# heiheishuang/MuDG

Hardware: AMD Instinct MI355X
Metric: DDIM denoise steps/sec, MDM1024 576x1024x16f (CFG: 2 UNet forwards + fused update per step, per clip) (higher is better)
Workload: dtype bf16; 1 GPU; MDM1024 latents (B=1,4,16,72,128) + c_concat 8ch, context (B,333,1024), 50-step uniform_trailing DDIM schedule, cfg 7.5, guidance_rescale 0.7, eta 1.0, v-prediction, dynamic rescale; clips_per_gpu=1, parallelism=clip-DP x1 (no in-step collective), launch=hipGraph replay of each UNet pass (cond+uncond batched)

## Files before the change

### include/mudg_hip.h

```cpp
#ifndef MUDG_HIP_H
#define MUDG_HIP_H

#include <stdint.h>

#ifdef __cplusplus
extern "C" {
#endif

#define MUDG_OK          0
#define MUDG_EINVAL     -1
#define MUDG_ELAUNCH    -2
#define MUDG_EUNSUPPORTED -3

int mudg_version(void);
int mudg_operand_dtype(void);
const char* mudg_last_error(void);

typedef struct MudgGemmDesc {
    const void* X;
    const void* X2;
    const void* W;
    void*       Y;
    const float* bias;
    const float* gbias;
// ... 35 lines not shown
    int Nk2, ldk2, ldvt2, kv_div2;
    int64_t svt2;
    const void* Q8; const void* K8; const void* Qs; const void* Ks;
    int ldq8, ldk8, ldqs, ldks;
    int q_prescaled;
    float* Lse;
} MudgAttnDesc;
int mudg_attention(const MudgAttnDesc* d, void* stream);
int mudg_quantize_mxfp8(const void* X, int ldx, int64_t rows, int cols, void* Y8, int ldy, void* S, int lds, void* stream);

int mudg_temporal_attention(const void* QKV, void* O, int B, int T, int HW, int heads,
                            int ldqkv, int ldo, float scale, void* stream);
int mudg_temporal_self_attention_ok(int T, int HW, int heads, int C, int64_t ldx, int64_t ldw, int64_t ldo);
int mudg_temporal_self_attention(const void* X, const void* Wh, void* O, int B, int T, int HW, int heads, int C, int64_t ldx,
                                 int64_t ldw, int64_t ldo, float scale, void* stream);

int64_t mudg_groupnorm_ws_floats(int samples, int groups, int rows);
int mudg_groupnorm(const void* X, const void* X2, int csplit, int ldx, int ldx2, int x_fp32,
                   const float* gamma, const float* beta, void* Y, int ldy,
                   int samples, int rows, int C, int groups, float eps, int silu,
                   float* ws, void* stream);
int mudg_groupnorm_fused(const void* X, const void* X2, int csplit, int ldx, int ldx2, int x_fp32,
                         const float* gamma, const float* beta, void* Y, int ldy,
                         int samples, int rows, int C, int groups, float eps, int silu,
                         const float* P1, const float* P2, float* ws, void* stream);

int mudg_groupnorm_fused_rows(const void* X, const void* X2, int csplit, int ldx, int ldx2, int x_fp32,
                              const float* gamma, const float* beta, void* Y, int ldy,
                              int samples, int rows, int C, int groups, float eps, int silu,
                              const float* P1, int p1_rows, const float* P2, int p2_rows, float* ws, void* stream);
// ... 200 lines not shown
```

### mudg_amd/csrc/attention.hip

```cpp
#include "attn_shared.h"
#include <cstdlib>

namespace {

#if MUDG_PLANES == 1
template <bool TWO>
__global__ __launch_bounds__(256, 2) void attn_kernel(const MudgAttnDesc p, const int nqt, const int total) {
    __shared__ __attribute__((aligned(16))) h16 Ks[2 * ATILE];
    __shared__ __attribute__((aligned(16))) h16 Vs[2 * ATILE];

    const int tid = threadIdx.x, lane = tid & 63, wave = tid >> 6;
    const int l31 = lane & 31, hi = lane >> 5;

    const int w = xcd_work_item(total);
    const int pair = w / nqt, qt = w - pair * nqt;
    const int f = pair / p.heads, h = pair - f * p.heads;
    const h16* Qp = reinterpret_cast<const h16*>(p.Q) + (int64_t)f * p.Nq * p.ldq + h * 64;
    h16* Op = reinterpret_cast<h16*>(p.O) + (int64_t)f * p.Nq * p.ldo + h * 64;

    const int q = qt * QB + wave * 32 + l31;
    const bool qok = q < p.Nq;

    h16x8 qf[1][4];
    load_q_frags(qf[0], Qp, q, p.ldq, 0, qok, hi);
// ... 18 lines not shown

        for (int kt = 0; kt < nkt; ++kt) {
            const int cur = kt & 1;
            const bool more = kt + 1 < nkt;
            if (more) load_kv_tile(kv, kt + 1, lrow, kc, kr, vr);
            FLASH_TILE(Ks + cur * ATILE, Vs + cur * ATILE, qf, kt, kv.Nk, c, m_run, l_run, o, l31, hi);
            if (more) stage_padded(Ks + (cur ^ 1) * ATILE, Vs + (cur ^ 1) * ATILE, lrow, kc, kr, vr);
            __syncthreads();
        }
        inv = finish_set<TWO>(p, set, f, h, q, qok, hi, c, m_run, l_run, o, res);
    }
    if (qok) store_o16(o, inv, Op + (int64_t)q * p.ldo, hi, p.accumulate);
}

constexpr int XK_TILES = 3;
template <bool TWO>
__global__ __launch_bounds__(256, 2) void xattn_kernel(const MudgAttnDesc p, const int nqt, const int xq, const int nqc, const int total) {
    extern __shared__ __attribute__((aligned(16))) h16 xlds[];
    h16* Ks = xlds;
    h16* Vs = xlds + XK_TILES * ATILE;
    const int tid = threadIdx.x, lane = tid & 63, wave = tid >> 6;
    const int l31 = lane & 31, hi = lane >> 5;
    const int w = xcd_work_item(total);
    const int pair = w / nqc, qc = w - pair * nqc;
    const int f = pair / p.heads, h = pair - f * p.heads;
    const h16* Qp = reinterpret_cast<const h16*>(p.Q) + (int64_t)f * p.Nq * p.ldq + h * 64;
    h16* Op = reinterpret_cast<h16*>(p.O) + (int64_t)f * p.Nq * p.ldo + h * 64;
    const int nt0 = (p.Nk + KB - 1) / KB;

    {
        const int lrow = tid >> 3, kc = tid & 7;
#pragma unroll
// ... 17 lines not shown
        const int q = qt * QB + wave * 32 + l31;
        const bool qok = q < p.Nq;
        h16x8 qf[1][4];
        load_q_frags(qf[0], Qp, q, p.ldq, 0, qok, hi);
        f32x16 o[2], res[TWO ? 2 : 1];
        float inv = 0.f;
#pragma unroll
        for (int set = 0; set < (TWO ? 2 : 1); ++set) {
            const int Nk = set == 0 ? p.Nk : p.Nk2;
#pragma unroll
            for (int r = 0; r < 16; ++r) { o[0][r] = 0.f; o[1][r] = 0.f; }
            float m_run = -INFINITY, l_run = 0.f;
            const int nkt = (Nk + KB - 1) / KB;
            for (int kt = 0; kt < nkt; ++kt) {
                const int ti = set == 0 ? kt : nt0 + kt;
                FLASH_TILE(Ks + ti * ATILE, Vs + ti * ATILE, qf, kt, Nk, c, m_run, l_run, o, l31, hi);
            }
            inv = finish_set<TWO>(p, set, f, h, q, qok, hi, c, m_run, l_run, o, res);
        }
        if (qok) store_o16(o, inv, Op + (int64_t)q * p.ldo, hi, p.accumulate);
    }
}

__global__ __launch_bounds__(256, 2) void attn64q_kernel(const MudgAttnDesc p, const int nqt, const int total) {
    __shared__ __attribute__((aligned(16))) h16 Ks[2 * ATILE];
    __shared__ __attribute__((aligned(16))) h16 Vs[2 * ATILE];

    const int tid = threadIdx.x, lane = tid & 63, wave = tid >> 6;
    const int l31 = lane & 31, hi = lane >> 5;
    const int w = xcd_work_item(total);
    const int pair = w / nqt, qt = w - pair * nqt;
    const int f = pair / p.heads, h = pair - f * p.heads;
    const KvSet kv = kv_set(p, f, h, 0);

    const h16* Qp = reinterpret_cast<const h16*>(p.Q) + (int64_t)f * p.Nq * p.ldq + h * 64;
    h16* Op = reinterpret_cast<h16*>(p.O) + (int64_t)f * p.Nq * p.ldo + h * 64;
// ... 374 lines not shown
        if (rok) {
            h16* dst = O + row * ldo + h * 64 + dp * DW;
#pragma unroll
            for (int i = 0; i < DW / 8; ++i) {
                h16x8 t;
#pragma unroll
                for (int e = 0; e < 8; ++e) t[e] = (h16)ov[i * 8 + e];
                st16(dst + i * 8, as_u32x4(t));
            }
        }
    }
}


#if MUDG_PLANES == 1
#ifdef MUDG_OPERAND_FP16
typedef __attribute__((ext_vector_type(4))) _Float16 mf4;
#define MFMA_16x16x32(a, b, c) __builtin_amdgcn_mfma_f32_16x16x32_f16(a, b, c, 0, 0, 0)
#define MFMA_16x16x16(a, b, c) __builtin_amdgcn_mfma_f32_16x16x16f16(a, b, c, 0, 0, 0)
#else
typedef __attribute__((ext_vector_type(4))) short mf4;
#define MFMA_16x16x32(a, b, c) __builtin_amdgcn_mfma_f32_16x16x32_bf16(a, b, c, 0, 0, 0)
#define MFMA_16x16x16(a, b, c) __builtin_amdgcn_mfma_f32_16x16x16bf16_1k(a, b, c, 0, 0, 0)
#endif

__device__ __forceinline__ int tattn_fz(int rg) { return (rg & 1) | ((rg >> 1) << 3); }
__device__ __forceinline__ void tattn_item_mfma(const char* qs, const char* ks, const char* vs, const int c, const int g, const int T,
                                                const float scale, float (&ov)[16]) {
    f32x4 st = {0.f, 0.f, 0.f, 0.f};
#pragma unroll
    for (int s = 0; s < 2; ++s) {
        const int off = c * 128 + (((g + 4 * s) ^ (c & 7)) << 4);
        st = MFMA_16x16x32(as_h16x8(ld16(ks + off)), as_h16x8(ld16(qs + off)), st);
    }

    float sc[4];
    float mx = -INFINITY;
#pragma unroll
    for (int i = 0; i < 4; ++i) { sc[i] = (4 * g + i < T) ? st[i] * scale : -INFINITY; mx = fmaxf(mx, sc[i]); }
// ... 680 lines not shown
        }
        else if (dma_ok && d.q_prescaled && lean) hipLaunchKernelGGL((attn64d_kernel<true, false>), dim3((unsigned)total2), dim3(256), 0, s, d, nqt2, (int)total2);
        else if (dma_ok) hipLaunchKernelGGL((attn64d_kernel<false, false>), dim3((unsigned)total2), dim3(256), 0, s, d, nqt2, (int)total2);
        else hipLaunchKernelGGL(attn64q_kernel, dim3((unsigned)total2), dim3(256), 0, s, d, nqt2, (int)total2);
    } else {
        static int xv = -1;
        if (xv < 0) xv = mudg_variant("ATTN_X", 1);
        int xq = (int)(total / 1024);
        xq = xq > 8 ? 8 : xq;
        if (xv && xq >= 2 && d.Nk <= 2 * KB && (!d.K2 || d.Nk2 <= KB)) {
            constexpr int smem = 2 * XK_TILES * ATILE * (int)sizeof(h16);
            if (const int rc = mudg_lds_opt_in<&xattn_kernel<false>>(smem, "mudg_attention")) return rc;
            if (const int rc = mudg_lds_opt_in<&xattn_kernel<true>>(smem, "mudg_attention")) return rc;
            const int nqc = (nqt + xq - 1) / xq;
            const int64_t totx = (int64_t)nqc * d.F * d.heads;
            if (d.K2) hipLaunchKernelGGL(xattn_kernel<true>, dim3((unsigned)totx), dim3(256), smem, s, d, nqt, xq, nqc, (int)totx);
            else hipLaunchKernelGGL(xattn_kernel<false>, dim3((unsigned)totx), dim3(256), smem, s, d, nqt, xq, nqc, (int)totx);
        }
        else if (d.K2) hipLaunchKernelGGL(attn_kernel<true>, dim3((unsigned)total), dim3(256), 0, s, d, nqt, (int)total);
        else hipLaunchKernelGGL(attn_kernel<false>, dim3((unsigned)total), dim3(256), 0, s, d, nqt, (int)total);
    }
#endif
    const int rc = mudg_check_launch("mudg_attention");
    const double bh = (double)d.F * d.heads;
    mudg_prof_end(slot, s, 4.0 * bh * d.Nq * (double)(d.Nk + (d.K2 ? d.Nk2 : 0)) * 64.0,
                  bh * (2.0 * d.Nq + 2.0 * d.Nk / d.kv_div + (d.K2 ? 2.0 * d.Nk2 / d.kv_div2 : 0.0)) * 64.0 * 2.0);
    return rc;
}

#if MUDG_PLANES == 1
namespace {
__global__ __launch_bounds__(256) void quantize_mxfp8_kernel(const h16* __restrict__ X, int ldx, int64_t rows, int nblk,
// ... 107 lines not shown
    const int rc0 = mudg_lds_opt_in<tsattn_fused_kernel>(TSA_LDS, "mudg_temporal_self_attention");
    if (rc0 != MUDG_OK) return rc0;
    hipStream_t s = reinterpret_cast<hipStream_t>(stream);
    const int slot = mudg_prof_begin(MUDG_FAM_GEMM, s);
    hipLaunchKernelGGL(tsattn_fused_kernel, dim3((unsigned)total), dim3(256), TSA_LDS, s, (const h16*)X, (const h16*)Wh, (h16*)O, HW, heads, C,
                       ldx, ldw, ldo, scale, (int)total);
    const int rc = mudg_check_launch("mudg_temporal_self_attention");
    const double M = (double)B * T * HW;
    mudg_prof_end(slot, s, 2.0 * M * 3.0 * C * C + 4.0 * (double)B * HW * heads * T * T * 64.0, (2.0 * M * C + 3.0 * C * C) * 2.0);
    return rc;
#else
    (void)X; (void)Wh; (void)O; (void)B; (void)T; (void)HW; (void)heads; (void)C; (void)ldx; (void)ldw; (void)ldo; (void)scale; (void)stream;
    MUDG_FAIL(MUDG_EUNSUPPORTED, "mudg_temporal_self_attention: the fused kernel belongs to the 16-bit operand builds");
#endif
}
```

### mudg_amd/csrc/attn_shared.h

```cpp
#pragma once
#include "common.h"
#include <type_traits>

constexpr int QB = 128;
constexpr int KB = 64;
constexpr int ALD = 72;
constexpr int ATILE = 64 * ALD;

struct KvSet {
    const h16* Kp;
    const h16* Vp;
    int Nk, ldk, ldvt;
    int psk, psv;
};
__device__ __forceinline__ KvSet kv_set(const MudgAttnDesc& p, int f, int h, int set) {
    KvSet kv;
    if (set == 0) {
        kv.Kp = reinterpret_cast<const h16*>(p.K) + (int64_t)(f / p.kv_div) * p.Nk * p.ldk + h * 64;
        kv.Vp = reinterpret_cast<const h16*>(p.Vt) + (int64_t)(f / p.kv_div) * p.svt + (int64_t)(h * 64) * p.ldvt;
        kv.Nk = p.Nk; kv.ldk = p.ldk; kv.ldvt = p.ldvt;
    } else {
        kv.Kp = reinterpret_cast<const h16*>(p.K2) + (int64_t)(f / p.kv_div2) * p.Nk2 * p.ldk2 + h * 64;
        kv.Vp = reinterpret_cast<const h16*>(p.Vt2) + (int64_t)(f / p.kv_div2) * p.svt2 + (int64_t)(h * 64) * p.ldvt2;
        kv.Nk = p.Nk2; kv.ldk = p.ldk2; kv.ldvt = p.ldvt2;
// ... 29 lines not shown
                }
            }
            vr[pl][i] = v;
        }
}
__device__ __forceinline__ void stage_padded(h16* Kt, h16* Vt, int lrow, int kc, const u32x4 (&kr)[PLANES][2], const u32x4 (&vr)[PLANES][2]) {
#pragma unroll
    for (int pl = 0; pl < PLANES; ++pl)
#pragma unroll
        for (int i = 0; i < 2; ++i) {
            st16(&Kt[pl * ATILE + (lrow + 32 * i) * ALD + kc * 8], kr[pl][i]);
            st16(&Vt[pl * ATILE + (lrow + 32 * i) * ALD + kc * 8], vr[pl][i]);
        }
}

__device__ __forceinline__ void mask_ragged(f32x16 (&s)[2], int kt, int Nk, int hi) {
    if (kt * KB + KB > Nk) {
#pragma unroll
        for (int sub = 0; sub < 2; ++sub)
#pragma unroll
            for (int r = 0; r < 16; ++r) {
                const int j = kt * KB + sub * 32 + (r & 3) + 8 * (r >> 2) + 4 * hi;
                if (j >= Nk) s[sub][r] = -INFINITY;
            }
    }
}

__device__ __forceinline__ float row_max32(const f32x16 (&s)[2]) {
    float mx = s[0][0];
#pragma unroll
    for (int r = 1; r < 16; ++r) mx = fmaxf(mx, s[0][r]);
#pragma unroll
    for (int r = 0; r < 16; ++r) mx = fmaxf(mx, s[1][r]);
    return fmaxf(mx, __shfl_xor(mx, 32, 64));
}

__device__ __forceinline__ void put_p(h16x8 (&pk)[PLANES][2][2], int sub, int r, float e) {
    h16 piece[PLANES];
    split_operand(e, piece);
#pragma unroll
    for (int pl = 0; pl < PLANES; ++pl) pk[pl][sub][r >> 3][r & 7] = piece[pl];
}

__device__ __forceinline__ void softmax_step_classic(const f32x16 (&s)[2], float c, float& m_run, float& l_run, f32x16 (&o)[2],
                                                     h16x8 (&pk)[PLANES][2][2]) {
    const float mx = row_max32(s);
    const bool grew = !__all(mx <= m_run);
    const float m_new = grew ? fmaxf(m_run, mx) : m_run;
    const float alpha = grew ? __builtin_amdgcn_exp2f((m_run - m_new) * c) : 1.0f;
    const float mc = m_new * c;
    m_run = m_new;
    float ps = 0.f;
#pragma unroll
    for (int sub = 0; sub < 2; ++sub)
#pragma unroll
        for (int r = 0; r < 16; ++r) {
            const float e = __builtin_amdgcn_exp2f(fmaf(s[sub][r], c, -mc));
            ps += e;
            put_p(pk, sub, r, e);
        }
    l_run = l_run * alpha + ps;
    if (grew) {
#pragma unroll
        for (int r = 0; r < 16; ++r) { o[0][r] *= alpha; o[1][r] *= alpha; }
    }
}

#ifdef MUDG_OPERAND_FP16
constexpr float LEAN_LIMIT = 32768.f;
// ... 11 lines not shown
            put_p(pk, sub, r, e);
        }
    l_run += ps;
    return !(ps <= LEAN_LIMIT);
}
template <bool LEAN, class KeyLoop>
__device__ __forceinline__ void lean_or_classic(const bool& overflow, KeyLoop key_loop) {
    if constexpr (LEAN) {
        key_loop(std::true_type{});
        if (__syncthreads_or(overflow ? 1 : 0)) key_loop(std::false_type{});
    } else {
        key_loop(std::false_type{});
    }
}

#define FLASH_TILE(Kt, Vt, qf, kt, Nk, c, m_run, l_run, o, l31, hi) do {                                                  \
    const h16* const ft_K = (Kt); const h16* const ft_V = (Vt); const int ft_kt = (kt), ft_Nk = (Nk);                     \
    f32x16 ft_s[2];                                                                                                       \
    _Pragma("unroll") for (int sub = 0; sub < 2; ++sub) {                                                                 \
        _Pragma("unroll") for (int r = 0; r < 16; ++r) ft_s[sub][r] = 0.f;                                                \
        _Pragma("unroll") for (int sg = 0; sg < NSEG; ++sg) {                                                             \
            const h16* kp = ft_K + seg_xp(sg) * ATILE + (sub * 32 + (l31)) * ALD + (hi) * 8;                              \
            _Pragma("unroll") for (int ks = 0; ks < 4; ++ks) {                                                            \
                const h16x8 kf = *reinterpret_cast<const h16x8*>(kp + ks * 16);                                           \
                ft_s[sub] = MFMA_32x32x16(kf, (qf)[seg_wp(sg)][ks], ft_s[sub]);                                           \
            }                                                                                                             \
        }                                                                                                                 \
    }                                                                                                                     \
    mask_ragged(ft_s, ft_kt, ft_Nk, (hi));                                                                                \
    h16x8 ft_pk[PLANES][2][2];                                                                                            \
    softmax_step_classic(ft_s, (c), (m_run), (l_run), (o), ft_pk);                                                        \
    _Pragma("unroll") for (int dt = 0; dt < 2; ++dt)                                                                      \
        _Pragma("unroll") for (int sg = 0; sg < NSEG; ++sg) {                                                             \
            const h16* vp = ft_V + seg_xp(sg) * ATILE + (dt * 32 + (l31)) * ALD + 4 * (hi);                               \
            _Pragma("unroll") for (int sub = 0; sub < 2; ++sub)                                                           \
                _Pragma("unroll") for (int jj = 0; jj < 2; ++jj) {                                                        \
                    const int kk = sub * 32 + jj * 16;                                                                    \
                    const h16x4 lo = *reinterpret_cast<const h16x4*>(vp + kk);                                            \
                    const h16x4 up = *reinterpret_cast<const h16x4*>(vp + kk + 8);                                        \
                    h16x8 vf;                                                                                             \
                    _Pragma("unroll") for (int e = 0; e < 4; ++e) { vf[e] = lo[e]; vf[4 + e] = up[e]; }                   \
                    (o)[dt] = MFMA_32x32x16(vf, ft_pk[seg_wp(sg)][sub][jj], (o)[dt]);                                     \
                }                                                                                                         \
        }                                                                                                                 \
} while (0)

__device__ __forceinline__ void store_lse(const MudgAttnDesc& p, int f, int h, int q, bool qok, int hi, float c, float m_run, float l_tot) {
    if (p.Lse && qok && hi == 0) p.Lse[((int64_t)f * p.Nq + q) * p.heads + h] = m_run * c + __log2f(l_tot);
}
__device__ __forceinline__ void store_o16(const f32x16 (&o)[2], float inv, h16* orow, int hi, int accumulate) {
#pragma unroll
    for (int dt = 0; dt < 2; ++dt)
#pragma unroll
        for (int g = 0; g < 4; ++g) {
            h16* dst = orow + dt * 32 + 8 * g + 4 * hi;
            float v[4];
#pragma unroll
            for (int j = 0; j < 4; ++j) v[j] = o[dt][4 * g + j] * inv;
            if (accumulate) {
                Pack8 old; old.u = *reinterpret_cast<const u32x2*>(dst);
// ... 53 lines not shown
```

### mudg_amd/engine/unet.py

```python
import torch
import torch.nn as nn

from .. import ops
from . import packing as pk



import os as _os
_LEAN_ATTENTION = _os.environ.get("MUDG_ATTN_LEAN", "1") != "0"
_TCONV_SLAB = _os.environ.get("MUDG_TCONV_SLAB", "1") != "0"
_TSATTN_FUSED = _os.environ.get("MUDG_TSATTN_FUSED", "1") != "0"
_FP8_ATTENTION = _os.environ.get("MUDG_ATTN_FP8", "0") == "1"


class _Ctx:
    __slots__ = ("B", "T", "emb", "text", "img", "n_text", "n_img", "img_div", "kv_cache", "replicas", "skips")

    def __init__(self):
        self.replicas, self.skips = 1, None

    def fan_out(self, rows):
        r, self.replicas = self.replicas, 1
        self.B *= r
        self.emb = self.emb.repeat(r, 1)
        if self.skips is not None:
            self.skips[:] = [(ops.repeat_rows(t, r), h, w) for t, h, w in self.skips]
# ... 81 lines not shown
        skip = _linear(mod.skip_connection, ops.cast_bf16(x), x2=None if x2 is None else ops.cast_bf16(x2), stream=True, hw=hw)
    out = _conv3x3(mod.out_layers[3], a, frames, h, w, residual=skip, stream=True)
    if mod.use_temporal_conv:
        out = temporal_conv_block(mod.temopral_conv, out, ctx, hw)
    return out


def _cross_kv(attn, ctx):
    k_text = ops.gemm(ctx.text, pk.linear(attn.to_k))
    vt_text, ld_text = _vt_projection(attn.to_v, ctx.text, ctx.B, ctx.n_text)
    if ctx.img is None or not attn.image_cross_attention:
        return k_text, vt_text, ld_text, None, None, 0
    k_img = ops.gemm(ctx.img, pk.linear(attn.to_k_ip))
    vt_img, ld_img = _vt_projection(attn.to_v_ip, ctx.img, ctx.img.shape[0] // ctx.n_img, ctx.n_img)
    return k_text, vt_text, ld_text, k_img, vt_img, ld_img


def spatial_block(blk, hcur, frames, hw, ctx, last):
    a1, a2 = blk.attn1, blk.attn2
    c, heads = hcur.shape[1], a1.heads
    n1 = _ln(blk.norm1, hcur)
    lean = _LEAN_ATTENTION and ops.hip.planes() <= 2
    wqk = pk.qk_prescaled(a1, a1.to_q, a1.to_k, a1.scale) if lean else pk.linear_cat(a1, "qk", (a1.to_q, a1.to_k))
    use_fp8 = lean and ops.hip.planes() == 1 and _FP8_ATTENTION and hw >= 512 and hw % 64 == 0
    fp8 = None
    if use_fp8:
        qk, q8, s8 = ops.gemm(n1, wqk, fp8=True)
        fp8 = (q8[:, :c], s8[:, :c // 32], q8[:, c:], s8[:, c // 32:])
    else:
        qk = ops.gemm(n1, wqk, frame_rows=hw)
    vt, ldv = _vt_projection(a1.to_v, n1, frames, hw)
    att = ops.empty_rows(frames * hw, c, ops.H16(), hcur.device)
    ops.attention(qk[:, :c], qk[:, c:], vt, att, frames=frames, heads=heads, nq=hw, nk=hw, ldvt=ldv, svt=c * ldv,
                  scale=a1.scale, q_prescaled=lean, fp8=fp8)
    hcur = _linear(a1.to_out[0], att, residual=hcur, stream=True, hw=hw)
    if ctx.replicas > 1:
        hcur = ctx.fan_out(hcur)
        frames = ctx.B * ctx.T
    n2 = _ln(blk.norm2, hcur)
    q2 = ops.gemm(n2, pk.linear(a2.to_q), frame_rows=hw)
    key = id(a2)
    if key not in ctx.kv_cache:
        ctx.kv_cache[key] = _cross_kv(a2, ctx)
    k_text, vt_text, ld_text, k_img, vt_img, ld_img = ctx.kv_cache[key]
    att2 = ops.empty_rows(frames * hw, c, ops.H16(), hcur.device)
    if k_img is not None and a2.image_cross_attention_scale != 1.0:
        raise NotImplementedError("image_cross_attention_scale != 1.0")
    ops.attention(q2, k_text, vt_text, att2, frames=frames, heads=heads, nq=hw, nk=ctx.n_text, ldvt=ld_text,
                  svt=c * ld_text, kv_div=ctx.T, scale=a2.scale, k2=k_img, vt2=vt_img, nk2=ctx.n_img,
                  ldvt2=ld_img if k_img is not None else None, svt2=c * ld_img if k_img is not None else None,
                  kv_div2=ctx.img_div)
    hcur = _linear(a2.to_out[0], att2, residual=hcur, stream=True, hw=hw)
    return _feed_forward(blk.ff, _ln(blk.norm3, hcur), hcur, stream=not last, hw=hw)


def spatial_transformer(mod, x, h, w, ctx):
    hw = h * w
    cur = _linear(mod.proj_in, _gn(mod.norm, x, None, ctx.B * ctx.T, hw, False), stream=True, hw=hw)
    n = len(mod.transformer_blocks)
    for i, blk in enumerate(mod.transformer_blocks):
        shared = ctx.replicas
        cur = spatial_block(blk, cur, ctx.B * ctx.T, hw, ctx, i == n - 1)
        if ctx.replicas != shared:
            x = ops.repeat_rows(x, shared)
    return _linear(mod.proj_out, cur, residual=x, stream=True, stats=True, hw=hw)

# ... 254 lines not shown
```

### mudg_amd/hip.py

```python
from __future__ import annotations

import ctypes as C
import os

_HERE = os.path.dirname(os.path.abspath(__file__))
LIB_PATHS = {"bf16": os.path.join(_HERE, "libmudg_hip.so"), "fp16": os.path.join(_HERE, "libmudg_hip_fp16.so"),
             "bf16x3": os.path.join(_HERE, "libmudg_hip_x3.so"), "bf16x6": os.path.join(_HERE, "libmudg_hip_x6.so")}
_MODES = {"bf16": (0, 1), "fp16": (1, 1), "bf16x3": (2, 2), "bf16x6": (3, 3)}
_operand = os.environ.get("MUDG_OPERAND", "bf16").lower()
LIB_PATH = LIB_PATHS["bf16"]


def set_operand(name: str) -> None:
    global _operand
    name = name.lower()
    if name not in LIB_PATHS:
        raise MudgError(f"unknown operand type {name!r} ({' | '.join(LIB_PATHS)})")
    if _lib is not None and name != _operand:
        raise MudgError("the operand type must be chosen before the first kernel call")
    _operand = name


def operand_name() -> str:
    return _operand
# ... 85 lines not shown


_P, _I, _L, _F, _D = C.c_void_p, C.c_int, C.c_int64, C.c_float, C.c_double
SIGNATURES = {
    "mudg_version": (_I, []),
    "mudg_operand_dtype": (_I, []),
    "mudg_last_error": (C.c_char_p, []),
    "mudg_gemm": (_I, [C.POINTER(GemmDesc), _P]),
    "mudg_gemm_stats_rows": (_I, [C.POINTER(GemmDesc)]),
    "mudg_conv_subpixel_ok": (_I, [C.POINTER(GemmDesc)]),
    "mudg_attention": (_I, [C.POINTER(AttnDesc), _P]),
    "mudg_quantize_mxfp8": (_I, [_P, _I, _L, _I, _P, _I, _P, _I, _P]),
    "mudg_temporal_attention": (_I, [_P, _P, _I, _I, _I, _I, _I, _I, _F, _P]),
    "mudg_temporal_self_attention_ok": (_I, [_I, _I, _I, _I, _L, _L, _L]),
    "mudg_temporal_self_attention": (_I, [_P, _P, _P, _I, _I, _I, _I, _I, _L, _L, _L, _F, _P]),
    "mudg_groupnorm_ws_floats": (_L, [_I, _I, _I]),
    "mudg_groupnorm": (_I, [_P, _P, _I, _I, _I, _I, _P, _P, _P, _I, _I, _I, _I, _I, _F, _I, _P, _P]),
    "mudg_groupnorm_fused": (_I, [_P, _P, _I, _I, _I, _I, _P, _P, _P, _I, _I, _I, _I, _I, _F, _I, _P, _P, _P, _P]),
    "mudg_groupnorm_fused_rows": (_I, [_P, _P, _I, _I, _I, _I, _P, _P, _P, _I, _I, _I, _I, _I, _F, _I, _P, _I, _P, _I, _P, _P]),
    "mudg_layernorm": (_I, [_P, _I, _I, _P, _P, _P, _I, _I, _I, _F, _P]),
    "mudg_softmax_rows": (_I, [_P, _I, _P, _I, _I, _I, _P]),
    "mudg_timestep_embedding": (_I, [_P, _P, _P, _I, _I, _P]),
    "mudg_small_linear": (_I, [_P, _P, _I, _P, _P, _I, _I, _I, _I, _I, _I, _P]),
    "mudg_ncthw_to_rows": (_I, [_P, _I, _P, _I, _I, _I, _I, _I, _I, _I, _I, _P]),
    "mudg_rows_to_ncthw": (_I, [_P, _I, _I, _I, _P, _I, _I, _I, _I, _I, _F, _I, _I, _P]),
    "mudg_cast_f32_bf16": (_I, [_P, _P, _L, _P]),
    "mudg_cast_rows": (_I, [_P, _I, _L, _P, _I, _L, _L, _L, _P]),
    "mudg_zero_channels": (_I, [_P, _I, _I, _I, _I, _P]),
    "mudg_copy_rows": (_I, [_P, _L, _P, _L, _L, _L, _P]),
    "mudg_axpy_f32": (_I, [_P, _P, _L, _F, _P]),
# ... 137 lines not shown
```

### mudg_amd/ops.py

```python
from __future__ import annotations

import ctypes as C
import math
from typing import Optional

import torch

from . import hip



def H16():
    return hip.operand_dtype()


def STREAM():
    import os
    if hip.operand_name() != "bf16" or os.environ.get("MUDG_STREAM", "").lower() == "fp32":
        return torch.float32
    return torch.float16


def kind(t) -> int:
    if t.dtype == torch.float32:
# ... 247 lines not shown
    rows, cols = x.shape
    y = torch.empty((rows, cols), dtype=torch.uint8, device=x.device)
    sc = torch.empty((rows, cols // 32), dtype=torch.uint8, device=x.device)
    hip.check(hip.lib().mudg_quantize_mxfp8(x.data_ptr(), x.stride(0), rows, cols, y.data_ptr(), y.stride(0), sc.data_ptr(),
                                            sc.stride(0), _stream()), "mudg_quantize_mxfp8")
    return y, sc


def temporal_attention(qkv, out, *, clips, t, hw, heads, scale=0.125):
    hip.check(hip.lib().mudg_temporal_attention(qkv.data_ptr(), out.data_ptr(), clips, t, hw, heads,
                                                qkv.stride(0), out.stride(0), scale, _stream()),
              "mudg_temporal_attention")
    return out


def temporal_self_attention_ok(t, hw, heads, c, ldx=None, ldw=None, ldo=None):
    return bool(hip.lib().mudg_temporal_self_attention_ok(t, hw, heads, c, c if ldx is None else ldx, c if ldw is None else ldw,
                                                          c if ldo is None else ldo))


def temporal_self_attention(x, wh, out, *, clips, t, hw, heads, scale=0.125):
    _rows(x); _rows(wh); _rows(out)
    rows, c = x.shape
    if rows != clips * t * hw or tuple(out.shape) != (rows, c) or tuple(wh.shape) != (3 * c, c):
        raise hip.MudgError(f"temporal_self_attention: x {tuple(x.shape)}, wh {tuple(wh.shape)}, out {tuple(out.shape)} are not "
                            f"[clips * t * hw = {clips * t * hw}][C], [3C][C], [clips * t * hw][C]")
    _drop_stats(out)
    hip.check(hip.lib().mudg_temporal_self_attention(x.data_ptr(), wh.data_ptr(), out.data_ptr(), clips, t, hw, heads, x.shape[1],
                                                     x.stride(0), wh.stride(0), out.stride(0), scale, _stream()),
              "mudg_temporal_self_attention")
# ... 884 lines not shown
```

Measured before the change: 8.694 steps/s.

## Fuse Q projection into spatial cross-attention kernel and skip empty key sub-tiles

Adds a fused kernel that computes the query projection (X·Wq per head) with MFMA into LDS and then runs flash cross-attention over the preloaded text/image K/V tiles. This removes a separate GEMM launch and the round trip of the Q tensor through global memory, for channels up to 256. The flash tile is also templated so that tiles whose second 32-key sub-block is fully out of range compute only one sub-block. The cost is recomputing the Q projection per head with a serial K loop inside the attention grid, and extra LDS pressure.

```diff
diff --git a/include/mudg_hip.h b/include/mudg_hip.h
--- a/include/mudg_hip.h
+++ b/include/mudg_hip.h
@@ -73,6 +73,8 @@
 int mudg_temporal_self_attention_ok(int T, int HW, int heads, int C, int64_t ldx, int64_t ldw, int64_t ldo);
 int mudg_temporal_self_attention(const void* X, const void* Wh, void* O, int B, int T, int HW, int heads, int C, int64_t ldx,
                                  int64_t ldw, int64_t ldo, float scale, void* stream);
+int mudg_cross_attention_q_ok(const MudgAttnDesc* d, int C, int64_t ldx, int64_t ldw);
+int mudg_cross_attention_q(const MudgAttnDesc* d, const void* X, int64_t ldx, const void* Wq, int64_t ldw, int C, void* stream);
 
 int64_t mudg_groupnorm_ws_floats(int samples, int groups, int rows);
 int mudg_groupnorm(const void* X, const void* X2, int csplit, int ldx, int ldx2, int x_fp32,
diff --git a/mudg_amd/csrc/attention.hip b/mudg_amd/csrc/attention.hip
--- a/mudg_amd/csrc/attention.hip
+++ b/mudg_amd/csrc/attention.hip
@@ -56,8 +56,13 @@
 }
 
 constexpr int XK_TILES = 3;
+#define XFLASH_TILE(Kt, Vt, qf, kt, Nk, all_subs, c, m_run, l_run, o, l31, hi) do {                                       \
+    if ((all_subs) || (kt) * KB + 32 < (Nk)) FLASH_TILE_N(2, Kt, Vt, qf, kt, Nk, c, m_run, l_run, o, l31, hi);            \
+    else FLASH_TILE_N(1, Kt, Vt, qf, kt, Nk, c, m_run, l_run, o, l31, hi);                                                \
+} while (0)
 template <bool TWO>
-__global__ __launch_bounds__(256, 2) void xattn_kernel(const MudgAttnDesc p, const int nqt, const int xq, const int nqc, const int total) {
+__global__ __launch_bounds__(256, 2) void xattn_kernel(const MudgAttnDesc p, const int nqt, const int xq, const int nqc, const int total,
+                                                       const int all_subs) {
     extern __shared__ __attribute__((aligned(16))) h16 xlds[];
     h16* Ks = xlds;
     h16* Vs = xlds + XK_TILES * ATILE;
@@ -105,12 +110,144 @@
             const int nkt = (Nk + KB - 1) / KB;
             for (int kt = 0; kt < nkt; ++kt) {
                 const int ti = set == 0 ? kt : nt0 + kt;
-                FLASH_TILE(Ks + ti * ATILE, Vs + ti * ATILE, qf, kt, Nk, c, m_run, l_run, o, l31, hi);
+                XFLASH_TILE(Ks + ti * ATILE, Vs + ti * ATILE, qf, kt, Nk, all_subs, c, m_run, l_run, o, l31, hi);
             }
             inv = finish_set<TWO>(p, set, f, h, q, qok, hi, c, m_run, l_run, o, res);
         }
         if (qok) store_o16(o, inv, Op + (int64_t)q * p.ldo, hi, p.accumulate);
     }
+}
+
+#ifdef MUDG_OPERAND_FP16
+typedef __attribute__((ext_vector_type(4))) _Float16 mf4;
+#define MFMA_16x16x32(a, b, c) __builtin_amdgcn_mfma_f32_16x16x32_f16(a, b, c, 0, 0, 0)
+#define MFMA_16x16x16(a, b, c) __builtin_amdgcn_mfma_f32_16x16x16f16(a, b, c, 0, 0, 0)
+#else
+typedef __attribute__((ext_vector_type(4))) short mf4;
+#define MFMA_16x16x32(a, b, c) __builtin_amdgcn_mfma_f32_16x16x32_bf16(a, b, c, 0, 0, 0)
+#define MFMA_16x16x16(a, b, c) __builtin_amdgcn_mfma_f32_16x16x16bf16_1k(a, b, c, 0, 0, 0)
+#endif
+constexpr int XF_KT = 32;
+constexpr int XF_STAGE = (QB + 64) * XF_KT * 2;
+constexpr int XF_KV = 2 * XK_TILES * ATILE * (int)sizeof(h16);
+constexpr int XF_LDS = XF_KV + 2 * XF_STAGE;
+static_assert(2 * XF_STAGE >= 4 * 32 * 128, "the dead stages must hold 4 waves x 32 rows x 128 B of q");
+static_assert(2 * XF_LDS <= 160 * 1024, "two workgroups per CU");
+template <bool TWO>
+__global__ __launch_bounds__(256, 2) void xattn_fused_kernel(const MudgAttnDesc p, const h16* __restrict__ X, const h16* __restrict__ W,
+                                                             const int64_t ldx, const int64_t ldw, const int C, const int nqt,
+                                                             const int total) {
+    extern __shared__ __attribute__((aligned(16))) h16 xlds[];
+    h16* Ks = xlds;
+    h16* Vs = xlds + XK_TILES * ATILE;
+    char* stages = reinterpret_cast<char*>(xlds) + XF_KV;
+    const int tid = threadIdx.x, lane = tid & 63, wave = tid >> 6;
+    const int l31 = lane & 31, hi = lane >> 5;
+    const int mc = lane & 15, mg = lane >> 4;
+    const int item = xcd_work_item(total);
+    const int tile = item / p.heads, h = item - tile * p.heads;
+    const int f = tile / nqt, qt = tile - f * nqt;
+    const int nt0 = (p.Nk + KB - 1) / KB;
+
+    const int lrow = tid >> 2, lch = tid & 3;
+    const h16* src[3];
+    bool xok[2];
+#pragma unroll
+    for (int i = 0; i < 2; ++i) {
+        const int r = qt * QB + lrow + 64 * i;
+        xok[i] = r < p.Nq;
+        src[i] = X + ((int64_t)f * p.Nq + (xok[i] ? r : 0)) * ldx + lch * 8;
+    }
+    src[2] = W + (int64_t)(h * 64 + lrow) * ldw + lch * 8;
+    const int soff = lrow * 64 + ((lch ^ ((lrow >> 2) & 3)) << 4);
+
+    u32x4 nx[3];
+    auto fetch = [&](int kt) {
+        nx[0] = xok[0] ? ld16(src[0] + kt * XF_KT) : zero16();
+        nx[1] = xok[1] ? ld16(src[1] + kt * XF_KT) : zero16();
+        nx[2] = ld16(src[2] + kt * XF_KT);
+    };
+    auto stage = [&](char* st) {
+#pragma unroll
+        for (int i = 0; i < 3; ++i) st16(st + soff + 4096 * i, nx[i]);
+    };
+
+    fetch(0);
+    {
+        const int krow = tid >> 3, kc = tid & 7;
+#pragma unroll
+        for (int set = 0; set < (TWO ? 2 : 1); ++set) {
+            const KvSet kv = kv_set(p, f, h, set);
+            const int nkt = (kv.Nk + KB - 1) / KB;
+            for (int kt = 0; kt < nkt; ++kt) {
+                const int ti = set == 0 ? kt : nt0 + kt;
+                u32x4 kr[1][2], vr[1][2];
+                load_kv_tile(kv, kt, krow, kc, kr, vr);
+                stage_padded(Ks + ti * ATILE, Vs + ti * ATILE, krow, kc, kr, vr);
+            }
+        }
+    }
+    stage(stages);
+    __syncthreads();
+
+    f32x4 acc[2][4];
+#pragma unroll
+    for (int pi = 0; pi < 2; ++pi)
+#pragma unroll
+        for (int nb = 0; nb < 4; ++nb) acc[pi][nb] = f32x4{0.f, 0.f, 0.f, 0.f};
+    const int foff = mc * 64 + ((mg ^ ((mc >> 2) & 3)) << 4);
+    const int nk = C / XF_KT;
+    for (int kt = 0; kt < nk; ++kt) {
+        const char* cur = stages + (kt & 1) * XF_STAGE;
+        if (kt + 1 < nk) fetch(kt + 1);
+        const h16x8 xf0 = as_h16x8(ld16(cur + (32 * wave) * 64 + foff));
+        const h16x8 xf1 = as_h16x8(ld16(cur + (32 * wave + 16) * 64 + foff));
+#pragma unroll
+        for (int nb = 0; nb < 4; ++nb) {
+            const h16x8 wf = as_h16x8(ld16(cur + (QB + 16 * nb) * 64 + foff));
+            acc[0][nb] = MFMA_16x16x32(wf, xf0, acc[0][nb]);
+            acc[1][nb] = MFMA_16x16x32(wf, xf1, acc[1][nb]);
+        }
+        if (kt + 1 < nk) stage(stages + ((kt + 1) & 1) * XF_STAGE);
+        __syncthreads();
+    }
+
+    char* mine = stages + wave * (32 * 128);
+#pragma unroll
+    for (int pi = 0; pi < 2; ++pi)
+#pragma unroll
+        for (int nb = 0; nb < 4; ++nb) {
+            Pack8 t;
+#pragma unroll
+            for (int i = 0; i < 4; ++i) t.h[i] = (h16)acc[pi][nb][i];
+            const int r = 16 * pi + mc;
+            *reinterpret_cast<u32x2*>(mine + r * 128 + (((2 * nb + (mg >> 1)) ^ (r & 7)) << 4) + ((mg & 1) << 3)) = t.u;
+        }
+    __builtin_amdgcn_wave_barrier();
+    h16x8 qf[1][4];
+#pragma unroll
+    for (int ks = 0; ks < 4; ++ks) qf[0][ks] = as_h16x8(ld16(mine + l31 * 128 + (((2 * ks + hi) ^ (l31 & 7)) << 4)));
+
+    const int q = qt * QB + wave * 32 + l31;
+    const bool qok = q < p.Nq;
+    h16* Op = reinterpret_cast<h16*>(p.O) + (int64_t)f * p.Nq * p.ldo + h * 64;
+    const float c = p.scale * 1.4426950408889634f;
+    f32x16 o[2], res[TWO ? 2 : 1];
+    float inv = 0.f;
+#pragma unroll
+    for (int set = 0; set < (TWO ? 2 : 1); ++set) {
+        const int Nk = set == 0 ? p.Nk : p.Nk2;
+#pragma unroll
+        for (int r = 0; r < 16; ++r) { o[0][r] = 0.f; o[1][r] = 0.f; }
+        float m_run = -INFINITY, l_run = 0.f;
+        const int nkt = (Nk + KB - 1) / KB;
+        for (int kt = 0; kt < nkt; ++kt) {
+            const int ti = set == 0 ? kt : nt0 + kt;
+            XFLASH_TILE(Ks + ti * ATILE, Vs + ti * ATILE, qf, kt, Nk, 0, c, m_run, l_run, o, l31, hi);
+        }
+        inv = finish_set<TWO>(p, set, f, h, q, qok, hi, c, m_run, l_run, o, res);
+    }
+    if (qok) store_o16(o, inv, Op + (int64_t)q * p.ldo, hi, 0);
 }
 
 __global__ __launch_bounds__(256, 2) void attn64q_kernel(const MudgAttnDesc p, const int nqt, const int total) {
@@ -515,15 +652,6 @@
 
 
 #if MUDG_PLANES == 1
-#ifdef MUDG_OPERAND_FP16
-typedef __attribute__((ext_vector_type(4))) _Float16 mf4;
-#define MFMA_16x16x32(a, b, c) __builtin_amdgcn_mfma_f32_16x16x32_f16(a, b, c, 0, 0, 0)
-#define MFMA_16x16x16(a, b, c) __builtin_amdgcn_mfma_f32_16x16x16f16(a, b, c, 0, 0, 0)
-#else
-typedef __attribute__((ext_vector_type(4))) short mf4;
-#define MFMA_16x16x32(a, b, c) __builtin_amdgcn_mfma_f32_16x16x32_bf16(a, b, c, 0, 0, 0)
-#define MFMA_16x16x16(a, b, c) __builtin_amdgcn_mfma_f32_16x16x16bf16_1k(a, b, c, 0, 0, 0)
-#endif
 
 __device__ __forceinline__ int tattn_fz(int rg) { return (rg & 1) | ((rg >> 1) << 3); }
 __device__ __forceinline__ void tattn_item_mfma(const char* qs, const char* ks, const char* vs, const int c, const int g, const int T,
@@ -1234,8 +1362,9 @@
             if (const int rc = mudg_lds_opt_in<&xattn_kernel<true>>(smem, "mudg_attention")) return rc;
             const int nqc = (nqt + xq - 1) / xq;
             const int64_t totx = (int64_t)nqc * d.F * d.heads;
-            if (d.K2) hipLaunchKernelGGL(xattn_kernel<true>, dim3((unsigned)totx), dim3(256), smem, s, d, nqt, xq, nqc, (int)totx);
-            else hipLaunchKernelGGL(xattn_kernel<false>, dim3((unsigned)totx), dim3(256), smem, s, d, nqt, xq, nqc, (int)totx);
+            const int all_subs = mudg_variant("ATTN_XSUB", 1) == 0;
+            if (d.K2) hipLaunchKernelGGL(xattn_kernel<true>, dim3((unsigned)totx), dim3(256), smem, s, d, nqt, xq, nqc, (int)totx, all_subs);
+            else hipLaunchKernelGGL(xattn_kernel<false>, dim3((unsigned)totx), dim3(256), smem, s, d, nqt, xq, nqc, (int)totx, all_subs);
         }
         else if (d.K2) hipLaunchKernelGGL(attn_kernel<true>, dim3((unsigned)total), dim3(256), 0, s, d, nqt, (int)total);
         else hipLaunchKernelGGL(attn_kernel<false>, dim3((unsigned)total), dim3(256), 0, s, d, nqt, (int)total);
@@ -1373,3 +1502,52 @@
     MUDG_FAIL(MUDG_EUNSUPPORTED, "mudg_temporal_self_attention: the fused kernel belongs to the 16-bit operand builds");
 #endif
 }
+
+extern "C" int mudg_cross_attention_q_ok(const MudgAttnDesc* d, int C, int64_t ldx, int64_t ldw) {
+#if MUDG_PLANES == 1
+    if (!d || d->F <= 0 || d->heads <= 0 || d->Nq <= 0 || C != d->heads * 64) return 0;
+    if (d->Nk <= 0 || d->Nk > 2 * KB || d->kv_div < 1 || d->F % d->kv_div != 0) return 0;
+    if (d->accumulate || d->Lse || d->Q8 || d->q_prescaled) return 0;
+    if (ldx % 8 != 0 || ldw % 8 != 0 || d->ldk % 8 != 0 || d->ldvt % 8 != 0 || d->ldo % 8 != 0 || (d->svt & 7) != 0) return 0;
+    if (ldx < C || ldw < C || d->ldk < C || d->ldo < C || d->ldvt < d->Nk) return 0;
+    if (d->K2 || d->Vt2) {
+        if (!d->K2 || !d->Vt2 || d->Nk2 <= 0 || d->Nk2 > KB || d->kv_div2 < 1 || d->F % d->kv_div2 != 0) return 0;
+        if (d->ldk2 % 8 != 0 || d->ldvt2 % 8 != 0 || (d->svt2 & 7) != 0 || d->ldk2 < C || d->ldvt2 < d->Nk2) return 0;
+    }
+    return 1;
+#else
+    (void)d; (void)C; (void)ldx; (void)ldw;
+    return 0;
+#endif
+}
+
+extern "C" int mudg_cross_attention_q(const MudgAttnDesc* dp, const void* X, int64_t ldx, const void* Wq, int64_t ldw, int C, void* stream) {
+#if MUDG_PLANES == 1
+    MUDG_REQUIRE(dp, "mudg_cross_attention_q: null descriptor");
+    const MudgAttnDesc d = *dp;
+    MUDG_REQUIRE(X && Wq && d.K && d.Vt && d.O, "mudg_cross_attention_q: null pointer");
+    MUDG_REQUIRE(aligned16(X) && aligned16(Wq) && aligned16(d.K) && aligned16(d.Vt) && aligned16(d.O) && aligned16(d.K2) && aligned16(d.Vt2),
+                 "mudg_cross_attention_q: alignment");
+    if (!mudg_cross_attention_q_ok(dp, C, ldx, ldw))
+        MUDG_FAIL(MUDG_EUNSUPPORTED, "mudg_cross_attention_q: heads=%d C=%d Nk=%d Nk2=%d outside the fused kernel (C = 64 heads, Nk <= 128, "
+                  "Nk2 <= 64, dense 16-byte rows, no accumulate / Lse / fp8 / prescaled q): project with mudg_gemm and call mudg_attention",
+                  d.heads, C, d.Nk, d.K2 ? d.Nk2 : 0);
+    const int nqt = (d.Nq + QB - 1) / QB;
+    const int64_t total = (int64_t)nqt * d.F * d.heads;
+    MUDG_REQUIRE(total < (1ll << 31), "mudg_cross_attention_q: grid too large");
+    if (const int rc = mudg_lds_opt_in<&xattn_fused_kernel<false>>(XF_LDS, "mudg_cross_attention_q")) return rc;
+    if (const int rc = mudg_lds_opt_in<&xattn_fused_kernel<true>>(XF_LDS, "mudg_cross_attention_q")) return rc;
+    hipStream_t s = reinterpret_cast<hipStream_t>(stream);
+    const int slot = mudg_prof_begin(MUDG_FAM_ATTN, s);
+    if (d.K2) hipLaunchKernelGGL(xattn_fused_kernel<true>, dim3((unsigned)total), dim3(256), XF_LDS, s, d, (const h16*)X, (const h16*)Wq, ldx, ldw, C, nqt, (int)total);
+    else hipLaunchKernelGGL(xattn_fused_kernel<false>, dim3((unsigned)total), dim3(256), XF_LDS, s, d, (const h16*)X, (const h16*)Wq, ldx, ldw, C, nqt, (int)total);
+    const int rc = mudg_check_launch("mudg_cross_attention_q");
+    const double M = (double)d.F * d.Nq, bh = (double)d.F * d.heads;
+    mudg_prof_end(slot, s, 2.0 * M * C * C + 4.0 * bh * d.Nq * (double)(d.Nk + (d.K2 ? d.Nk2 : 0)) * 64.0,
+                  (2.0 * M * C + (double)C * C) * 2.0 + bh * (2.0 * d.Nk / d.kv_div + (d.K2 ? 2.0 * d.Nk2 / d.kv_div2 : 0.0)) * 64.0 * 2.0);
+    return rc;
+#else
+    (void)dp; (void)X; (void)ldx; (void)Wq; (void)ldw; (void)C; (void)stream;
+    MUDG_FAIL(MUDG_EUNSUPPORTED, "mudg_cross_attention_q: the fused kernel belongs to the 16-bit operand builds");
+#endif
+}
diff --git a/mudg_amd/csrc/attn_shared.h b/mudg_amd/csrc/attn_shared.h
--- a/mudg_amd/csrc/attn_shared.h
+++ b/mudg_amd/csrc/attn_shared.h
@@ -67,10 +67,11 @@
         }
 }
 
-__device__ __forceinline__ void mask_ragged(f32x16 (&s)[2], int kt, int Nk, int hi) {
+template <int NS>
+__device__ __forceinline__ void mask_ragged(f32x16 (&s)[NS], int kt, int Nk, int hi) {
     if (kt * KB + KB > Nk) {
 #pragma unroll
-        for (int sub = 0; sub < 2; ++sub)
+        for (int sub = 0; sub < NS; ++sub)
 #pragma unroll
             for (int r = 0; r < 16; ++r) {
                 const int j = kt * KB + sub * 32 + (r & 3) + 8 * (r >> 2) + 4 * hi;
@@ -79,12 +80,15 @@
     }
 }
 
-__device__ __forceinline__ float row_max32(const f32x16 (&s)[2]) {
+template <int NS>
+__device__ __forceinline__ float row_max32(const f32x16 (&s)[NS]) {
     float mx = s[0][0];
 #pragma unroll
     for (int r = 1; r < 16; ++r) mx = fmaxf(mx, s[0][r]);
-#pragma unroll
-    for (int r = 0; r < 16; ++r) mx = fmaxf(mx, s[1][r]);
+    if constexpr (NS == 2) {
+#pragma unroll
+        for (int r = 0; r < 16; ++r) mx = fmaxf(mx, s[1][r]);
+    }
     return fmaxf(mx, __shfl_xor(mx, 32, 64));
 }
 
@@ -95,7 +99,8 @@
     for (int pl = 0; pl < PLANES; ++pl) pk[pl][sub][r >> 3][r & 7] = piece[pl];
 }
 
-__device__ __forceinline__ void softmax_step_classic(const f32x16 (&s)[2], float c, float& m_run, float& l_run, f32x16 (&o)[2],
+template <int NS>
+__device__ __forceinline__ void softmax_step_classic(const f32x16 (&s)[NS], float c, float& m_run, float& l_run, f32x16 (&o)[2],
                                                      h16x8 (&pk)[PLANES][2][2]) {
     const float mx = row_max32(s);
     const bool grew = !__all(mx <= m_run);
@@ -105,7 +110,7 @@
     m_run = m_new;
     float ps = 0.f;
 #pragma unroll
-    for (int sub = 0; sub < 2; ++sub)
+    for (int sub = 0; sub < NS; ++sub)
 #pragma unroll
         for (int r = 0; r < 16; ++r) {
             const float e = __builtin_amdgcn_exp2f(fmaf(s[sub][r], c, -mc));
@@ -147,10 +152,10 @@
     }
 }
 
-#define FLASH_TILE(Kt, Vt, qf, kt, Nk, c, m_run, l_run, o, l31, hi) do {                                                  \
+#define FLASH_TILE_N(NS, Kt, Vt, qf, kt, Nk, c, m_run, l_run, o, l31, hi) do {                                            \
     const h16* const ft_K = (Kt); const h16* const ft_V = (Vt); const int ft_kt = (kt), ft_Nk = (Nk);                     \
-    f32x16 ft_s[2];                                                                                                       \
-    _Pragma("unroll") for (int sub = 0; sub < 2; ++sub) {                                                                 \
+    f32x16 ft_s[NS];                                                                                                      \
+    _Pragma("unroll") for (int sub = 0; sub < NS; ++sub) {                                                                \
         _Pragma("unroll") for (int r = 0; r < 16; ++r) ft_s[sub][r] = 0.f;                                                \
         _Pragma("unroll") for (int sg = 0; sg < NSEG; ++sg) {                                                             \
             const h16* kp = ft_K + seg_xp(sg) * ATILE + (sub * 32 + (l31)) * ALD + (hi) * 8;                              \
@@ -166,7 +171,7 @@
     _Pragma("unroll") for (int dt = 0; dt < 2; ++dt)                                                                      \
         _Pragma("unroll") for (int sg = 0; sg < NSEG; ++sg) {                                                             \
             const h16* vp = ft_V + seg_xp(sg) * ATILE + (dt * 32 + (l31)) * ALD + 4 * (hi);                               \
-            _Pragma("unroll") for (int sub = 0; sub < 2; ++sub)                                                           \
+            _Pragma("unroll") for (int sub = 0; sub < NS; ++sub)                                                          \
                 _Pragma("unroll") for (int jj = 0; jj < 2; ++jj) {                                                        \
                     const int kk = sub * 32 + jj * 16;                                                                    \
                     const h16x4 lo = *reinterpret_cast<const h16x4*>(vp + kk);                                            \
@@ -177,6 +182,7 @@
                 }                                                                                                         \
         }                                                                                                                 \
 } while (0)
+#define FLASH_TILE(Kt, Vt, qf, kt, Nk, c, m_run, l_run, o, l31, hi) FLASH_TILE_N(2, Kt, Vt, qf, kt, Nk, c, m_run, l_run, o, l31, hi)
 
 __device__ __forceinline__ void store_lse(const MudgAttnDesc& p, int f, int h, int q, bool qok, int hi, float c, float m_run, float l_tot) {
     if (p.Lse && qok && hi == 0) p.Lse[((int64_t)f * p.Nq + q) * p.heads + h] = m_run * c + __log2f(l_tot);
diff --git a/mudg_amd/engine/unet.py b/mudg_amd/engine/unet.py
--- a/mudg_amd/engine/unet.py
+++ b/mudg_amd/engine/unet.py
@@ -10,6 +10,7 @@
 _LEAN_ATTENTION = _os.environ.get("MUDG_ATTN_LEAN", "1") != "0"
 _TCONV_SLAB = _os.environ.get("MUDG_TCONV_SLAB", "1") != "0"
 _TSATTN_FUSED = _os.environ.get("MUDG_TSATTN_FUSED", "1") != "0"
+_XATTN_FUSED = _os.environ.get("MUDG_XATTN_FUSED", "1") != "0"
 _FP8_ATTENTION = _os.environ.get("MUDG_ATTN_FP8", "0") == "1"
 
 
@@ -121,6 +122,14 @@
     k_img = ops.gemm(ctx.img, pk.linear(attn.to_k_ip))
     vt_img, ld_img = _vt_projection(attn.to_v_ip, ctx.img, ctx.img.shape[0] // ctx.n_img, ctx.n_img)
     return k_text, vt_text, ld_text, k_img, vt_img, ld_img
+
+
+_XATTN_MAX_C = 256
+
+
+def _xattn_fused(c, x, out, k, vt, kv):
+    return (_XATTN_FUSED and c <= _XATTN_MAX_C
+            and ops.cross_attention_q_ok(c, k, vt, ldx=x.stride(0), ldw=c, ldo=out.stride(0), **kv))
 
 
 def spatial_block(blk, hcur, frames, hw, ctx, last):
@@ -145,7 +154,6 @@
         hcur = ctx.fan_out(hcur)
         frames = ctx.B * ctx.T
     n2 = _ln(blk.norm2, hcur)
-    q2 = ops.gemm(n2, pk.linear(a2.to_q), frame_rows=hw)
     key = id(a2)
     if key not in ctx.kv_cache:
         ctx.kv_cache[key] = _cross_kv(a2, ctx)
@@ -153,10 +161,14 @@
     att2 = ops.empty_rows(frames * hw, c, ops.H16(), hcur.device)
     if k_img is not None and a2.image_cross_attention_scale != 1.0:
         raise NotImplementedError("image_cross_attention_scale != 1.0")
-    ops.attention(q2, k_text, vt_text, att2, frames=frames, heads=heads, nq=hw, nk=ctx.n_text, ldvt=ld_text,
-                  svt=c * ld_text, kv_div=ctx.T, scale=a2.scale, k2=k_img, vt2=vt_img, nk2=ctx.n_img,
-                  ldvt2=ld_img if k_img is not None else None, svt2=c * ld_img if k_img is not None else None,
-                  kv_div2=ctx.img_div)
+    kv = dict(frames=frames, heads=heads, nq=hw, nk=ctx.n_text, ldvt=ld_text, svt=c * ld_text, kv_div=ctx.T, scale=a2.scale,
+              k2=k_img, vt2=vt_img, nk2=ctx.n_img, ldvt2=ld_img if k_img is not None else None,
+              svt2=c * ld_img if k_img is not None else None, kv_div2=ctx.img_div)
+    if _xattn_fused(c, n2, att2, k_text, vt_text, kv):
+        ops.cross_attention_q(n2, pk.linear(a2.to_q), k_text, vt_text, att2, **kv)
+    else:
+        q2 = ops.gemm(n2, pk.linear(a2.to_q), frame_rows=hw)
+        ops.attention(q2, k_text, vt_text, att2, **kv)
     hcur = _linear(a2.to_out[0], att2, residual=hcur, stream=True, hw=hw)
     return _feed_forward(blk.ff, _ln(blk.norm3, hcur), hcur, stream=not last, hw=hw)
 
diff --git a/mudg_amd/hip.py b/mudg_amd/hip.py
--- a/mudg_amd/hip.py
+++ b/mudg_amd/hip.py
@@ -123,6 +123,8 @@
     "mudg_temporal_attention": (_I, [_P, _P, _I, _I, _I, _I, _I, _I, _F, _P]),
     "mudg_temporal_self_attention_ok": (_I, [_I, _I, _I, _I, _L, _L, _L]),
     "mudg_temporal_self_attention": (_I, [_P, _P, _P, _I, _I, _I, _I, _I, _L, _L, _L, _F, _P]),
+    "mudg_cross_attention_q_ok": (_I, [C.POINTER(AttnDesc), _I, _L, _L]),
+    "mudg_cross_attention_q": (_I, [C.POINTER(AttnDesc), _P, _L, _P, _L, _I, _P]),
     "mudg_groupnorm_ws_floats": (_L, [_I, _I, _I]),
     "mudg_groupnorm": (_I, [_P, _P, _I, _I, _I, _I, _P, _P, _P, _I, _I, _I, _I, _I, _F, _I, _P, _P]),
     "mudg_groupnorm_fused": (_I, [_P, _P, _I, _I, _I, _I, _P, _P, _P, _I, _I, _I, _I, _I, _F, _I, _P, _P, _P, _P]),
diff --git a/mudg_amd/ops.py b/mudg_amd/ops.py
--- a/mudg_amd/ops.py
+++ b/mudg_amd/ops.py
@@ -285,6 +285,46 @@
     return out
 
 
+def _cross_q_desc(k, vt, out_ptr, ldo, frames, heads, nq, nk, ldvt, svt, kv_div, scale, k2, vt2, nk2, ldvt2, svt2, kv_div2,
+                  accumulate=False, lse=False):
+    d = hip.AttnDesc()
+    d.K, d.Vt, d.O = k.data_ptr(), vt.data_ptr(), out_ptr
+    d.F, d.heads, d.Nq, d.Nk = frames, heads, nq, nk
+    d.ldk, d.ldvt, d.ldo = k.stride(0), vt.stride(0) if ldvt is None else ldvt, ldo
+    d.svt = heads * 64 * d.ldvt if svt is None else svt
+    d.kv_div, d.scale, d.accumulate = kv_div, scale, int(accumulate)
+    if lse:
+        d.Lse = 256
+    if k2 is not None:
+        d.K2, d.Vt2, d.Nk2, d.ldk2 = k2.data_ptr(), vt2.data_ptr(), nk2, k2.stride(0)
+        d.ldvt2 = vt2.stride(0) if ldvt2 is None else ldvt2
+        d.svt2 = heads * 64 * d.ldvt2 if svt2 is None else svt2
+        d.kv_div2 = kv_div2
+    return d
+
+
+def cross_attention_q_ok(c, k, vt, *, frames, heads, nq, nk, ldx=None, ldw=None, ldo=None, ldvt=None, svt=None, kv_div=1, scale=0.125,
+                         k2=None, vt2=None, nk2=0, ldvt2=None, svt2=None, kv_div2=1, accumulate=False, lse=False):
+    d = _cross_q_desc(k, vt, 256, c if ldo is None else ldo, frames, heads, nq, nk, ldvt, svt, kv_div, scale, k2, vt2, nk2, ldvt2, svt2,
+                      kv_div2, accumulate, lse)
+    return bool(hip.lib().mudg_cross_attention_q_ok(C.byref(d), c, c if ldx is None else ldx, c if ldw is None else ldw))
+
+
+def cross_attention_q(x, wq, k, vt, out, *, frames, heads, nq, nk, ldvt=None, svt=None, kv_div=1, scale=0.125,
+                      k2=None, vt2=None, nk2=0, ldvt2=None, svt2=None, kv_div2=1):
+    _rows(x); _rows(wq); _rows(out)
+    rows, c = x.shape
+    if rows != frames * nq or tuple(out.shape) != (rows, c) or tuple(wq.shape) != (c, c):
+        raise hip.MudgError(f"cross_attention_q: x {tuple(x.shape)}, wq {tuple(wq.shape)}, out {tuple(out.shape)} are not "
+                            f"[frames * nq = {frames * nq}][C], [C][C], [frames * nq][C]")
+    _drop_stats(out)
+    d = _cross_q_desc(k, vt, out.data_ptr(), out.stride(0), frames, heads, nq, nk, ldvt, svt, kv_div, scale, k2, vt2, nk2, ldvt2, svt2,
+                      kv_div2)
+    hip.check(hip.lib().mudg_cross_attention_q(C.byref(d), x.data_ptr(), x.stride(0), wq.data_ptr(), wq.stride(0), c, _stream()),
+              "mudg_cross_attention_q")
+    return out
+
+
 def temporal_self_attention_ok(t, hw, heads, c, ldx=None, ldw=None, ldo=None):
     return bool(hip.lib().mudg_temporal_self_attention_ok(t, hw, heads, c, c if ldx is None else ldx, c if ldw is None else ldw,
                                                           c if ldo is None else ldo))
```

Result: no change. 8.683 steps/s (-0.1%).
